# noway/nzcp-circom

Measured on NVIDIA B200. Metric: groth16_proofs_per_sec, higher is better.
Workload: dtype u256 (Fr/Fq Montgomery, 8x32-bit limbs, IMAD.WIDE carry chains)

## Files before the change

nzcp_circom_b200/csrc/msm.cu:

```cuda
#include <atomic>

#include "common.cuh"
#include "msm_pair.cuh"

#ifndef NZCP_G2_ACC_BLOCKS
#define NZCP_G2_ACC_BLOCKS 3
#endif

namespace nzcp {

#ifndef NZCP_TASK_LEN_MAX
#define NZCP_TASK_LEN_MAX 64
#endif
static constexpr int kTaskLenMax = NZCP_TASK_LEN_MAX;
static_assert((NZCP_TASK_LEN_MAX & (NZCP_TASK_LEN_MAX - 1)) == 0 && NZCP_TASK_LEN_MAX >= 8, "task length must be a power of two");
static constexpr int kTaskLenMin = 8;
#ifndef NZCP_TARGET_TASKS
#define NZCP_TARGET_TASKS (148 * 640)
#endif
static constexpr int kTargetTasks = NZCP_TARGET_TASKS;
#ifndef NZCP_HEAVY_TASKS
#define NZCP_HEAVY_TASKS 16
#endif
static constexpr int kHeavyTasks = NZCP_HEAVY_TASKS;
// ... 331 lines not shown
    for (int r = 0; r < C; r++) round_off[(size_t)r * pitch + n_buckets] = carry[r];
    flags[5] = carry[R];
  }
}

__global__ void __launch_bounds__(256)
msm_task_fill_kernel(const uint32_t* __restrict__ bcount, const uint32_t* __restrict__ offsets,
                     const uint32_t* __restrict__ task_off, uint2* __restrict__ tasks, uint32_t n_buckets,
                     const uint32_t* __restrict__ flags) {
  const uint32_t t = blockIdx.x * blockDim.x + threadIdx.x;
  if (t >= flags[2]) return;
  const uint32_t tl = flags[4];
  uint32_t lo = 0, hi = n_buckets;
  while (hi - lo > 1) {
    uint32_t mid = (lo + hi) >> 1;
    if (task_off[mid] <= t) lo = mid; else hi = mid;
  }
  (void)tl;
  const uint32_t k = task_off[lo + 1] - task_off[lo], j = t - task_off[lo];
  const uint32_t cnt = bcount[lo], base = cnt / k, rem = cnt % k;
  tasks[t] = make_uint2(offsets[lo] + j * base + (j < rem ? j : rem), base + (j < rem ? 1u : 0u));
}

template <class T>
__device__ __forceinline__ void prefetch_l1(const T* p) {
  asm volatile("prefetch.global.L1 [%0];" ::"l"(p));
  if (sizeof(T) > 64) asm volatile("prefetch.global.L1 [%0];" ::"l"(reinterpret_cast<const char*>(p) + 64));
}

template <class F> struct AccumOcc { static constexpr int kBlocks = 5; };
template <> struct AccumOcc<Fq2> { static constexpr int kBlocks = NZCP_G2_ACC_BLOCKS; };

template <class F>
__global__ void __launch_bounds__(128, AccumOcc<F>::kBlocks)
msm_accumulate_kernel(const Affine<F>* __restrict__ table, const uint32_t* __restrict__ entries,
                      const uint2* __restrict__ tasks, const uint32_t* __restrict__ flags, XYZZ<F>* __restrict__ partial, int pf) {
  uint32_t t = blockIdx.x * blockDim.x + threadIdx.x;
  if (t >= flags[2]) return;
  uint2 tk = tasks[t];
  XYZZ<F> acc = XYZZ<F>::inf();
  uint32_t e = entries[tk.x];
  if (pf & 1) prefetch_l1(table + (e & 0x7fffffffu));
  for (uint32_t k = 0; k < tk.y; k++) {
    uint32_t en = e;
    if (k + 1 < tk.y) {
      en = entries[tk.x + k + 1];
      if (pf & 1) prefetch_l1(table + (en & 0x7fffffffu));
    }
    Affine<F> q;
#if defined(__CUDA_ARCH__)
    if (sizeof(F) == sizeof(Fq) && (pf & 4)) q = gather_hinted<Affine<F>>(table + (e & 0x7fffffffu));
    else
#endif
      q = table[e & 0x7fffffffu];
    if (!q.is_inf()) xyzz_madd(acc, q, (e >> 31) != 0);
    e = en;
  }
  partial[t] = acc;
}

template <class F>
__global__ void __launch_bounds__(128, AccumOcc<F>::kBlocks)
msm_accumulate_pts_kernel(const Affine<F>* __restrict__ pts, const uint2* __restrict__ tasks,
                          const uint32_t* __restrict__ flags, XYZZ<F>* __restrict__ partial) {
  uint32_t t = blockIdx.x * blockDim.x + threadIdx.x;
  if (t >= flags[2]) return;
  uint2 tk = tasks[t];
  XYZZ<F> acc = XYZZ<F>::inf();
  for (uint32_t k = 0; k < tk.y; k++) {
    Affine<F> q = pts[tk.x + k];
    if (!q.is_inf()) xyzz_madd(acc, q, false);
  }
  partial[t] = acc;
}

static constexpr int kPairInvGroup = 32;
#ifndef NZCP_PAIR_FWD_BLOCKS
#define NZCP_PAIR_FWD_BLOCKS 1
#endif
template <class F, bool FROM_TABLE, int K>
__global__ void __launch_bounds__(128, (sizeof(F) == sizeof(Fq) ? NZCP_PAIR_FWD_BLOCKS : 1))
msm_pair_forward_kernel(const Affine<F>* __restrict__ src, const uint32_t* __restrict__ entries,
                        const uint32_t* __restrict__ off_in, const uint32_t* __restrict__ off_out, uint32_t n_buckets,
                        F* __restrict__ scratch, F* __restrict__ prod, int pf, Affine<F>* __restrict__ ops) {
  const uint32_t t = blockIdx.x * blockDim.x + threadIdx.x;
  PairSource<F, FROM_TABLE> ps{src, entries, pf};
  msm_pair_forward_body<F, FROM_TABLE, K>(t, gridDim.x * blockDim.x, ps, off_in, off_out, n_buckets, scratch, prod, ops);
}

template <class F, int K>
__global__ void __launch_bounds__(64)
msm_pair_invert_kernel(F* __restrict__ prod, const uint32_t* __restrict__ off_out, uint32_t n_buckets) {
  const uint32_t n_out = off_out[n_buckets];
  const uint32_t n_prod = pair_n_prod<K>(n_out);
  msm_pair_invert_body<F, kPairInvGroup>(blockIdx.x * blockDim.x + threadIdx.x, prod, n_prod);
}

template <class F, bool FROM_TABLE, int K>
__global__ void __launch_bounds__(128)
msm_pair_backward_kernel(const Affine<F>* __restrict__ src, const uint32_t* __restrict__ entries,
                         const uint32_t* __restrict__ off_in, const uint32_t* __restrict__ off_out, uint32_t n_buckets,
                         Affine<F>* __restrict__ dst, const F* __restrict__ scratch, const F* __restrict__ inv_prod, int pf,
                         const Affine<F>* __restrict__ ops) {
  const uint32_t t = blockIdx.x * blockDim.x + threadIdx.x;
  PairSource<F, FROM_TABLE> ps{src, entries, pf};
  msm_pair_backward_body<F, FROM_TABLE, K>(t, gridDim.x * blockDim.x, ps, off_in, off_out, n_buckets, dst, scratch, inv_prod,
                                           ops);
}

template <class T>
__device__ __forceinline__ T load_cg(const T* p) {
  static_assert(sizeof(T) % 16 == 0, "16-byte granules");
  T r;
  const uint4* s = reinterpret_cast<const uint4*>(p);
  uint4* d = reinterpret_cast<uint4*>(&r);
#pragma unroll
  for (int i = 0; i < (int)(sizeof(T) / 16); i++) d[i] = __ldcg(s + i);
  return r;
}

template <class T>
__device__ __forceinline__ T shfl_down_obj(const T& v, unsigned delta) {
  T r;
  const uint32_t* s = reinterpret_cast<const uint32_t*>(&v);
  uint32_t* d = reinterpret_cast<uint32_t*>(&r);
#pragma unroll
  for (int i = 0; i < (int)(sizeof(T) / 4); i++) d[i] = __shfl_down_sync(0xffffffffu, s[i], delta);
  return r;
}

template <class F>
__global__ void __launch_bounds__(128)
msm_combine_kernel(const uint32_t* __restrict__ task_off, const XYZZ<F>* __restrict__ partial,
                   XYZZ<F>* __restrict__ buckets, uint32_t n_buckets, uint32_t* __restrict__ heavy_list,
                   uint32_t* __restrict__ heavy_count) {
  const uint32_t b = blockIdx.x * blockDim.x + threadIdx.x;
  if (b >= n_buckets) return;
  const uint32_t t0 = task_off[b], nt = task_off[b + 1] - t0;
  if (nt > (uint32_t)kHeavyTasks) {
    heavy_list[atomicAdd(heavy_count, 1u)] = b;
    return;
  }
  XYZZ<F> acc = XYZZ<F>::inf();
  for (uint32_t j = 0; j < nt; j++) xyzz_add(acc, partial[t0 + j]);
  buckets[b] = acc;
}

__global__ void __launch_bounds__(1024)
msm_heavy_scan_kernel(const uint32_t* __restrict__ task_off, const uint32_t* __restrict__ heavy_list,
                      uint32_t* __restrict__ heavy_count, uint32_t* __restrict__ chunk_off) {
  __shared__ uint32_t sums[1024];
  const uint32_t n = heavy_count[0];
  const uint32_t per = (n + 1023) / 1024;
  const uint32_t b = threadIdx.x * per;
  const uint32_t e = b + per < n ? b + per : n;
  auto chunks = [&](uint32_t h) {
    uint32_t bk = heavy_list[h];
    return (task_off[bk + 1] - task_off[bk] + kHeavyChunk - 1) / kHeavyChunk;
  };
  uint32_t acc = 0;
  for (uint32_t h = b; h < e; h++) acc += chunks(h);
  sums[threadIdx.x] = acc;
  __syncthreads();
  for (int off = 1; off < 1024; off <<= 1) {
    uint32_t v = threadIdx.x >= (uint32_t)off ? sums[threadIdx.x - off] : 0;
    __syncthreads();
    sums[threadIdx.x] += v;
    __syncthreads();
  }
  uint32_t run = threadIdx.x ? sums[threadIdx.x - 1] : 0;
  for (uint32_t h = b; h < e; h++) {
    chunk_off[h] = run;
    run += chunks(h);
  }
  if (threadIdx.x == 1023) {
    chunk_off[n] = sums[1023];
    heavy_count[1] = sums[1023];
  }
}

template <class F>
__device__ __forceinline__ XYZZ<F> block_sum(XYZZ<F> acc, XYZZ<F>* sm) {
  sm[threadIdx.x] = acc;
  __syncthreads();
  for (uint32_t stride = blockDim.x / 2; stride >= 1; stride >>= 1) {
    if (threadIdx.x < stride) {
// ... 331 lines not shown
    const uint32_t n_ctr = nb * n_copies;
    DigitParams dp{n_copies, (uint32_t)n_points, s->table_free ? 0u : (uint32_t)s->n_points, s->c, s->n_windows,
                   (uint32_t)s->group_buckets, s->table_free ? (uint32_t)s->group_buckets : 0u, nb};
    const unsigned gp = div_up(n_points, 256);
    const size_t hist_bytes = (size_t)nb * sizeof(uint32_t);
    if (s->smem_hist) {
      NZCP_CUDA(cudaMemsetAsync(s->counts + n_ctr, 0, sizeof(uint32_t), st));
      msm_digits_smem_kernel<false><<<n_copies, sort_threads, hist_bytes, st>>>(scalars, dp, s->counts, nullptr, s->flags);
    } else {
      NZCP_CUDA(cudaMemsetAsync(s->counts, 0, (n_ctr + 1) * sizeof(uint32_t), st));
      msm_digits_kernel<false><<<gp, 256, 0, st>>>(scalars, dp, s->counts, nullptr, s->flags);
    }
    NZCP_LAUNCH_CHECK();
    const uint32_t n_scan = n_ctr + 1;
    const uint32_t n_blk = div_up(n_scan, kScanBlock);
    uint32_t* blk_sum = s->block_sums;
    uint32_t* blk_off = s->block_sums + (s->n_buckets * s->n_copies / kScanBlock + 2);
    msm_scan_sums_kernel<<<n_blk, 256, 0, st>>>(s->counts, blk_sum, n_scan);
    NZCP_LAUNCH_CHECK();
    msm_scan_kernel<false><<<1, 1024, 0, st>>>(blk_sum, blk_off, n_blk, s->flags + 3, s->flags);
    NZCP_LAUNCH_CHECK();
    msm_scan_apply_kernel<<<n_blk, 256, 0, st>>>(s->counts, blk_off, s->offsets, s->smem_hist ? nullptr : s->cursors, n_scan);
    NZCP_LAUNCH_CHECK();
    if (s->smem_hist)
      msm_digits_smem_kernel<true><<<n_copies, sort_threads, hist_bytes, st>>>(scalars, dp, s->offsets, s->entries, s->flags);
    else
      msm_digits_kernel<true><<<gp, 256, 0, st>>>(scalars, dp, s->cursors, s->entries, s->flags);
    NZCP_LAUNCH_CHECK();
    switch (s->rounds) {
      case 0: msm_round_plan_kernel<0><<<1, 1024, 0, st>>>(s->offsets, n_copies, nb, s->round_off, s->red_count, s->flags); break;
      case 1: msm_round_plan_kernel<1><<<1, 1024, 0, st>>>(s->offsets, n_copies, nb, s->round_off, s->red_count, s->flags); break;
      case 2: msm_round_plan_kernel<2><<<1, 1024, 0, st>>>(s->offsets, n_copies, nb, s->round_off, s->red_count, s->flags); break;
      default: msm_round_plan_kernel<3><<<1, 1024, 0, st>>>(s->offsets, n_copies, nb, s->round_off, s->red_count, s->flags); break;
    }
    NZCP_LAUNCH_CHECK();
    msm_scan_kernel<true><<<1, 1024, 0, st>>>(s->red_count, s->task_off, nb, s->flags + 2, s->flags);
    NZCP_LAUNCH_CHECK();
    msm_task_fill_kernel<<<div_up(s->max_tasks, 256), 256, 0, st>>>(s->red_count, s->round_off + (size_t)s->rounds * (nb + 1),
                                                                     s->task_off, s->tasks, nb, s->flags);
    NZCP_LAUNCH_CHECK();
  } else {
    NZCP_CUDA(cudaMemsetAsync(s->task_off, 0, (nb + 1) * sizeof(uint32_t), st));
  }
  NZCP_CUDA(cudaMemcpyAsync(s->flags_host, s->flags, 8 * sizeof(uint32_t), cudaMemcpyDeviceToHost, st));
}

uint32_t msm_sort_check(const MsmSort* s) {
  if (s->flags_host[1]) throw std::runtime_error("witness/scalar value is not a canonical field element (>= r)");
  return s->flags_host[3];
}

void msm_run_create(MsmRun* r, const MsmSort* sort, bool g2) {
  *r = MsmRun();
  r->g2 = g2;
  size_t psz = g2 ? sizeof(G2XYZZ) : sizeof(G1XYZZ);
  size_t tot = 0;
  if (g2) {
    NZCP_CUDA(cudaFuncSetAttribute(msm_combine_heavy_kernel<Fq2>, cudaFuncAttributeMaxDynamicSharedMemorySize,
                                   (int)(kHeavyThreads * sizeof(G2XYZZ))));
    NZCP_CUDA(cudaFuncSetAttribute(msm_combine_heavy2_kernel<Fq2>, cudaFuncAttributeMaxDynamicSharedMemorySize,
                                   (int)(kHeavyThreads * sizeof(G2XYZZ))));
    NZCP_CUDA(cudaFuncSetAttribute(msm_marginal_kernel<Fq2>, cudaFuncAttributeMaxDynamicSharedMemorySize,
                                   (int)(kMargThreads * sizeof(G2XYZZ))));
  }
  r->partial = dev_alloc<unsigned char>(sort->max_tasks * psz, &tot);
  r->buckets = dev_alloc<unsigned char>(sort->n_buckets * psz, &tot);
  r->n_groups = sort->n_groups;
  r->c = sort->c;
  r->marg = dev_alloc<unsigned char>((size_t)r->n_groups * kMaxDigits * 32 * psz, &tot);
  r->marg_done = dev_alloc<uint32_t>((size_t)r->n_groups * kMaxDigits, &tot);
  NZCP_CUDA(cudaMemset(r->marg_done, 0, (size_t)r->n_groups * kMaxDigits * sizeof(uint32_t)));
  r->result = dev_alloc<unsigned char>(psz, &tot);
  r->heavy_list = dev_alloc<uint32_t>(sort->n_buckets, &tot);
  r->heavy_count = dev_alloc<uint32_t>(2, &tot);
  r->chunk_off = dev_alloc<uint32_t>(sort->n_buckets + 1, &tot);
  r->chunk_partial = dev_alloc<unsigned char>((sort->max_tasks / kHeavyChunk + sort->n_buckets + 1) * psz, &tot);
  r->out = dev_alloc<unsigned char>((size_t)r->n_groups * (kMaxDigits + 1) * psz, &tot);
  NZCP_CUDA(cudaMallocHost(&r->out_host, (size_t)r->n_groups * (kMaxDigits + 1) * psz));
  memset(r->out_host, 0, (size_t)r->n_groups * (kMaxDigits + 1) * psz);
  r->n_digits = (sort->c - 1 + 4) / 5;
  NZCP_CUDA(cudaFuncSetAttribute(msm_sum_points_kernel<Fq2>, cudaFuncAttributeMaxDynamicSharedMemorySize,
                                 (int)(kHeavyThreads * sizeof(G2XYZZ))));
  if (sort->rounds > 0) {
    const size_t asz = g2 ? sizeof(G2Affine) : sizeof(G1Affine), fsz = asz / 2, pad = 128 * 64;
    r->round_pts[0] = dev_alloc<unsigned char>((sort->round_max[1] + pad) * asz, &tot);
    if (sort->rounds > 1) r->round_pts[1] = dev_alloc<unsigned char>((sort->round_max[2] + pad) * asz, &tot);
    r->round_prefix = dev_alloc<unsigned char>((sort->round_max[1] + pad) * fsz, &tot);
    if (g_tune_pair_stage.load())
      r->round_ops = dev_alloc<unsigned char>((sort->round_max[1] + pad) * 2 * asz, &tot);
    r->round_prod = dev_alloc<unsigned char>((sort->round_max[1] / 4 + pad) * fsz, &tot);
  }
  NZCP_CUDA(cudaEventCreate(&r->ev_acc0));
  NZCP_CUDA(cudaEventCreate(&r->ev_acc1));
  r->scratch_bytes = tot;
}

void msm_run_destroy(MsmRun* r) {
  cudaFree(r->partial);
  cudaFree(r->buckets);
  cudaFree(r->marg);
  cudaFree(r->marg_done);
  cudaFree(r->result);
  cudaFree(r->heavy_list);
  cudaFree(r->heavy_count);
  cudaFree(r->chunk_off);
  cudaFree(r->chunk_partial);
  cudaFree(r->out);
  cudaFree(r->round_pts[0]);
  cudaFree(r->round_pts[1]);
  cudaFree(r->round_prefix);
  cudaFree(r->round_ops);
  cudaFree(r->round_prod);
  if (r->out_host) cudaFreeHost(r->out_host);
  if (r->ev_acc0) cudaEventDestroy(r->ev_acc0);
  if (r->ev_acc1) cudaEventDestroy(r->ev_acc1);
  *r = MsmRun();
}

template <class F>
static void msm_run_launch_t(MsmRun* r, const MsmSort* s, const MsmTable* t, cudaStream_t st) {
  if (t->c != s->c || t->n_points != s->n_points || t->n_windows != (s->table_free ? 1 : s->n_windows))
    throw std::runtime_error("msm: table and sort plan do not match");
  const uint32_t nb = (uint32_t)s->n_buckets;
  const size_t psz = sizeof(XYZZ<F>);
  XYZZ<F>* partial = reinterpret_cast<XYZZ<F>*>(r->partial);
  XYZZ<F>* buckets = reinterpret_cast<XYZZ<F>*>(r->buckets);
  XYZZ<F>* out = reinterpret_cast<XYZZ<F>*>(r->out);
  NZCP_CUDA(cudaMemsetAsync(r->heavy_count, 0, 2 * sizeof(uint32_t), st));
  NZCP_CUDA(cudaEventRecord(r->ev_acc0, st));
  if (s->rounds == 0) {
    msm_accumulate_kernel<F><<<div_up(s->max_tasks, 128), 128, 0, st>>>(reinterpret_cast<const Affine<F>*>(t->pts),
                                                                       s->entries, s->tasks, s->flags, partial,
                                                                       (g_tune_acc_prefetch.load() ? 1 : 0) | (g_tune_gather_hint.load() ? 4 : 0));
    NZCP_LAUNCH_CHECK();
  } else {
    const Affine<F>* src = reinterpret_cast<const Affine<F>*>(t->pts);
    for (int rd = 1; rd <= s->rounds; rd++) {
      Affine<F>* dst = reinterpret_cast<Affine<F>*>(r->round_pts[(rd - 1) & 1]);
      const uint32_t* off_in = s->round_off + (size_t)(rd - 1) * (nb + 1);
      const uint32_t* off_out = s->round_off + (size_t)rd * (nb + 1);
      const int hint = g_tune_gather_hint.load() ? 4 : 0;
      const int pf_fwd = g_tune_pair_prefetch[0].load() | hint, pf_bwd = g_tune_pair_prefetch[1].load() | hint;
      int k = g_tune_pair_k[rd - 1].load();
      k = k >= 32 ? 32 : k >= 16 ? 16 : k >= 8 ? 8 : 4;
      const unsigned grid = div_up(div_up(s->round_max[rd], k) + kPairLanes, 128);
      const unsigned grid_inv = div_up(div_up((size_t)grid * 128, kPairInvGroup), 64);
      F* scratch = reinterpret_cast<F*>(r->round_prefix);
      F* prod = reinterpret_cast<F*>(r->round_prod);
      Affine<F>* ops = g_tune_pair_stage.load() ? reinterpret_cast<Affine<F>*>(r->round_ops) : nullptr;
#define NZCP_PAIR_LAUNCH(TABLE, KK)                                                                                       \
      do {                                                                                                                \
        msm_pair_forward_kernel<F, TABLE, KK><<<grid, 128, 0, st>>>(src, s->entries, off_in, off_out, nb, scratch, prod, \
                                                                    pf_fwd, TABLE ? ops : nullptr);                       \
        NZCP_LAUNCH_CHECK();                                                                                              \
        msm_pair_invert_kernel<F, KK><<<grid_inv, 64, 0, st>>>(prod, off_out, nb);                                        \
        NZCP_LAUNCH_CHECK();                                                                                              \
        msm_pair_backward_kernel<F, TABLE, KK><<<grid, 128, 0, st>>>(src, s->entries, off_in, off_out, nb, dst, scratch,  \
                                                                     prod, pf_bwd, TABLE ? ops : nullptr);                \
        NZCP_LAUNCH_CHECK();                                                                                              \
      } while (0)
      if (rd == 1) {
        if (k == 32) NZCP_PAIR_LAUNCH(true, 32); else if (k == 16) NZCP_PAIR_LAUNCH(true, 16);
        else if (k == 8) NZCP_PAIR_LAUNCH(true, 8); else NZCP_PAIR_LAUNCH(true, 4);
      } else {
        if (k == 32) NZCP_PAIR_LAUNCH(false, 32); else if (k == 16) NZCP_PAIR_LAUNCH(false, 16);
        else if (k == 8) NZCP_PAIR_LAUNCH(false, 8); else NZCP_PAIR_LAUNCH(false, 4);
      }
#undef NZCP_PAIR_LAUNCH
      src = dst;
    }
    msm_accumulate_pts_kernel<F><<<div_up(s->max_tasks, 128), 128, 0, st>>>(src, s->tasks, s->flags, partial);
    NZCP_LAUNCH_CHECK();
  }
  NZCP_CUDA(cudaEventRecord(r->ev_acc1, st));
  msm_combine_kernel<F><<<div_up(nb, 128), 128, 0, st>>>(s->task_off, partial, buckets, nb, r->heavy_list,
                                                                     r->heavy_count);
  NZCP_LAUNCH_CHECK();
  msm_heavy_scan_kernel<<<1, 1024, 0, st>>>(s->task_off, r->heavy_list, r->heavy_count, r->chunk_off);
  NZCP_LAUNCH_CHECK();
  XYZZ<F>* chunk_partial = reinterpret_cast<XYZZ<F>*>(r->chunk_partial);
  msm_combine_heavy_kernel<F><<<148 * 16, kHeavyThreads, kHeavyThreads * psz, st>>>(s->task_off, partial, r->heavy_list,
                                                                                    r->heavy_count, r->chunk_off, chunk_partial,
                                                                                    buckets);
  NZCP_LAUNCH_CHECK();
  msm_combine_heavy2_kernel<F><<<148, kHeavyThreads, kHeavyThreads * psz, st>>>(r->heavy_list, r->heavy_count, r->chunk_off,
                                                                                chunk_partial, buckets);
  NZCP_LAUNCH_CHECK();
  const uint32_t bits = (uint32_t)(s->c - 1);
  const uint32_t n_digits = (bits + 4) / 5;
  XYZZ<F>* marg = reinterpret_cast<XYZZ<F>*>(r->marg);
  msm_marginal_kernel<F><<<(unsigned)s->n_groups * n_digits * 32, kMargThreads, kMargThreads * psz, st>>>(buckets, marg, out,
                                                                                                      r->marg_done, bits, n_digits);
  NZCP_LAUNCH_CHECK();
  NZCP_CUDA(cudaMemcpyAsync(r->out_host, r->out, (size_t)s->n_groups * (n_digits + 1) * psz, cudaMemcpyDeviceToHost, st));
}

void msm_run_finish_device(MsmRun* r, cudaStream_t st) {
  if (r->g2)
    msm_finish_kernel<Fq2><<<1, 32, 0, st>>>(reinterpret_cast<const G2XYZZ*>(r->out), reinterpret_cast<G2XYZZ*>(r->result),
                                             (uint32_t)r->n_groups, (uint32_t)r->n_digits, r->c);
  else
    msm_finish_kernel<Fq><<<1, 32, 0, st>>>(reinterpret_cast<const G1XYZZ*>(r->out), reinterpret_cast<G1XYZZ*>(r->result),
                                            (uint32_t)r->n_groups, (uint32_t)r->n_digits, r->c);
  NZCP_LAUNCH_CHECK();
}

void msm_sum_points(const void* d_pts, uint32_t count, bool g2, void* d_result, cudaStream_t st) {
  if (g2) {
    NZCP_CUDA(cudaFuncSetAttribute(msm_sum_points_kernel<Fq2>, cudaFuncAttributeMaxDynamicSharedMemorySize,
                                   (int)(kHeavyThreads * sizeof(G2XYZZ))));
    msm_sum_points_kernel<Fq2><<<1, kHeavyThreads, kHeavyThreads * sizeof(G2XYZZ), st>>>(
        reinterpret_cast<const G2XYZZ*>(d_pts), count, reinterpret_cast<G2XYZZ*>(d_result));
  } else {
    msm_sum_points_kernel<Fq><<<1, kHeavyThreads, kHeavyThreads * sizeof(G1XYZZ), st>>>(
        reinterpret_cast<const G1XYZZ*>(d_pts), count, reinterpret_cast<G1XYZZ*>(d_result));
  }
  NZCP_LAUNCH_CHECK();
}

void msm_run_launch(MsmRun* r, const MsmSort* sort, const MsmTable* table, cudaStream_t st) {
  if (r->g2 != table->g2) throw std::runtime_error("msm: run and table group mismatch");
  if (r->g2)
    msm_run_launch_t<Fq2>(r, sort, table, st);
  else
    msm_run_launch_t<Fq>(r, sort, table, st);
}

template <class F>
static XYZZ<F> msm_run_finish_t(const MsmRun* r) {
  XYZZ<F> res = XYZZ<F>::inf();
  for (int g = r->n_groups - 1; g >= 0; g--) {
    const XYZZ<F>* w = reinterpret_cast<const XYZZ<F>*>(r->out_host) + (size_t)g * (r->n_digits + 1);
    XYZZ<F> acc = XYZZ<F>::inf();
    for (int k = r->n_digits - 1; k >= 0; k--) {
      if (!acc.is_inf())
        for (int d = 0; d < 5; d++) acc = xyzz_dbl(acc);
      xyzz_add(acc, w[k]);
    }
// ... 22 lines not shown
```

nzcp_circom_b200/csrc/msm_pair.cuh:

```cuda
#pragma once
#include "ec.cuh"


namespace nzcp {

enum PairKind { kPairNormal = 0, kPairDouble = 1, kPairFirst = 2, kPairSecond = 3, kPairInfinity = 4 };

#if defined(__CUDA_ARCH__)
template <class T>
__device__ __forceinline__ T gather_hinted(const T* p) {
  static_assert(sizeof(T) % 16 == 0, "16-byte granules");
  T r;
  uint4* d = reinterpret_cast<uint4*>(&r);
  const char* a = reinterpret_cast<const char*>(p);
#pragma unroll
  for (int i = 0; i < (int)(sizeof(T) / 16); i++)
    asm volatile("ld.global.nc.L2::64B.v4.u32 {%0, %1, %2, %3}, [%4];" : "=r"(d[i].x), "=r"(d[i].y), "=r"(d[i].z), "=r"(d[i].w) : "l"(a + 16 * i));
  return r;
}
#endif

template <class F, bool FROM_TABLE>
struct PairSource {
  const Affine<F>* pts;
  const uint32_t* entries;
  int pf = 0;
  HD uint32_t slot(uint32_t idx) const { return FROM_TABLE ? entries[idx] : idx; }
  HD F x_at(uint32_t slot) const {
#if defined(__CUDA_ARCH__)
    if (FROM_TABLE && (pf & 4)) return gather_hinted<F>(&pts[slot & 0x7fffffffu].x);
#endif
    return pts[FROM_TABLE ? (slot & 0x7fffffffu) : slot].x;
  }
  HD Affine<F> point_at(uint32_t slot) const {
    if (FROM_TABLE) {
      Affine<F> p;
#if defined(__CUDA_ARCH__)
      if (pf & 4) p = gather_hinted<Affine<F>>(&pts[slot & 0x7fffffffu]);
      else
#endif
        p = pts[slot & 0x7fffffffu];
      if (slot >> 31) p.y = f_neg(p.y);
      return p;
    }
    return pts[slot];
  }
  HD Affine<F> point(uint32_t idx) const { return point_at(slot(idx)); }
  HD void prefetch(uint32_t slot, bool whole_point) const {
#if defined(__CUDA_ARCH__)
    if ((pf & 3) == 0) return;
    const char* a = reinterpret_cast<const char*>(pts + (FROM_TABLE ? (slot & 0x7fffffffu) : slot));
    if ((pf & 3) == 1) {
      asm volatile("prefetch.global.L1 [%0];" ::"l"(a));
      if (sizeof(F) > 32 && whole_point) asm volatile("prefetch.global.L1 [%0];" ::"l"(a + 64));
    } else {
      asm volatile("prefetch.global.L2 [%0];" ::"l"(a));
      if (sizeof(F) > 32 && whole_point) asm volatile("prefetch.global.L2 [%0];" ::"l"(a + 64));
    }
#else
    (void)slot;
    (void)whole_point;
#endif
  }
};

struct PairWalk {
  const uint32_t* off_in;
  const uint32_t* off_out;
  uint32_t s, out0, out1, in0, len;
  HD void load() {
    out0 = off_out[s];
    out1 = off_out[s + 1];
    in0 = off_in[s];
    len = off_in[s + 1] - in0;
  }
  HD void forward_to(uint32_t o) {
    if (o < out1) return;
    do s++; while (o >= off_out[s + 1]);
    load();
  }
  HD void backward_to(uint32_t o) {
    if (o >= out0) return;
    do s--; while (o < off_out[s]);
    load();
  }
  HD uint32_t first(uint32_t o) const { return in0 + 2 * (o - out0); }
  HD bool paired(uint32_t o) const { return 2 * (o - out0) + 1 < len; }
};

template <class F>
HD int pair_classify(const Affine<F>& p1, const Affine<F>& p2, F& den) {
  if (p1.is_inf()) return kPairSecond;
  if (p2.is_inf()) return kPairFirst;
  den = f_sub(p2.x, p1.x);
  if (den.is_zero()) {
    if (p1.y == p2.y && !p1.y.is_zero()) {
      den = f_dbl(p1.y);
      return kPairDouble;
    }
    return kPairInfinity;
  }
  return kPairNormal;
}

static constexpr uint32_t kPairLanes = 32;
template <int K>
HD bool pair_thread_range(uint32_t t, const uint32_t* off_out, uint32_t n_buckets, uint32_t& o0, uint32_t& cnt) {
  const uint32_t n_out = off_out[n_buckets];
  const uint64_t first = (uint64_t)(t / kPairLanes) * (kPairLanes * K) + (t % kPairLanes);
  if (first >= n_out) return false;
  o0 = (uint32_t)first;
  const uint32_t left = (n_out - o0 + kPairLanes - 1) / kPairLanes;
  cnt = left < (uint32_t)K ? left : (uint32_t)K;
  return true;
}
template <int K>
HD uint32_t pair_n_prod(uint32_t n_out) {
  const uint32_t full = n_out / (kPairLanes * K), rem = n_out - full * (kPairLanes * K);
  return full * kPairLanes + (rem < kPairLanes ? rem : kPairLanes);
}
HD void pair_walk_seek(PairWalk& wk, uint32_t o, uint32_t n_buckets) {
  uint32_t lo = 0, hi = n_buckets;
  while (hi - lo > 1) {
    const uint32_t mid = (lo + hi) >> 1;
    if (wk.off_out[mid] <= o) lo = mid; else hi = mid;
  }
  wk.s = lo;
  wk.load();
}

template <class F, bool FROM_TABLE, int K>
HD void msm_pair_forward_body(uint32_t t, uint32_t stride, const PairSource<F, FROM_TABLE>& src, const uint32_t* off_in,
                              const uint32_t* off_out, uint32_t n_buckets, F* scratch, F* prod, Affine<F>* ops = nullptr) {
  uint32_t o0, cnt;
  if (!pair_thread_range<K>(t, off_out, n_buckets, o0, cnt)) return;
  PairWalk wk{off_in, off_out, 0, 0, 0, 0, 0};
  pair_walk_seek(wk, o0, n_buckets);
  F pre = F::one();
  bool have = false;
  bool pair_cur = wk.paired(o0);
  uint32_t a_cur = src.slot(wk.first(o0)), b_cur = pair_cur ? src.slot(wk.first(o0) + 1) : 0;
  for (uint32_t i = 0; i < cnt; i++) {
    bool pair_nxt = false;
    uint32_t a_nxt = 0, b_nxt = 0;
    if (i + 1 < cnt) {
      const uint32_t on = o0 + (i + 1) * kPairLanes;
      wk.forward_to(on);
      pair_nxt = wk.paired(on);
      if (pair_nxt || ops) a_nxt = src.slot(wk.first(on));
      if (pair_nxt) {
        b_nxt = src.slot(wk.first(on) + 1);
        src.prefetch(a_nxt, false);
        src.prefetch(b_nxt, false);
      }
    }
    if (ops) {
      const Affine<F> p1 = src.point_at(a_cur);
      const Affine<F> p2 = pair_cur ? src.point_at(b_cur) : Affine<F>::inf();
      ops[2 * ((size_t)i * stride + t)] = p1;
      ops[2 * ((size_t)i * stride + t) + 1] = p2;
      if (pair_cur) {
        F den;
        const int kind = pair_classify(p1, p2, den);
        if (kind == kPairNormal || kind == kPairDouble) {
          pre = have ? f_mul(pre, den) : den;
          have = true;
        }
      }
    } else if (pair_cur) {
      const F x1 = src.x_at(a_cur), x2 = src.x_at(b_cur);
      F den = f_sub(x2, x1);
      bool use = true;
      if (den.is_zero() || x1.is_zero() || x2.is_zero()) {
        const int kind = pair_classify(src.point_at(a_cur), src.point_at(b_cur), den);
        use = kind == kPairNormal || kind == kPairDouble;
      }
      if (use) {
        pre = have ? f_mul(pre, den) : den;
        have = true;
      }
    }
    scratch[(size_t)i * stride + t] = pre;
    pair_cur = pair_nxt;
    a_cur = a_nxt;
    b_cur = b_nxt;
  }
  prod[t] = pre;
}

template <class F, int KI>
HD void msm_pair_invert_body(uint32_t g, F* v, uint32_t n) {
  const uint32_t b = g * KI;
  if (b >= n) return;
  const uint32_t cnt = n - b < (uint32_t)KI ? n - b : (uint32_t)KI;
  F pre[KI];
  F run = v[b];
  pre[0] = run;
  for (uint32_t i = 1; i < cnt; i++) {
    run = f_mul(run, v[b + i]);
    pre[i] = run;
  }
  F inv = f_inv_fast(run);
  for (uint32_t i = cnt; i-- > 1;) {
    const F x = v[b + i];
    v[b + i] = f_mul(inv, pre[i - 1]);
    inv = f_mul(inv, x);
  }
  v[b] = inv;
}

template <class F>
HD Affine<F> pair_finish(const Affine<F>& p1, const Affine<F>& p2, F& inv, const F& before) {
  F den;
  const int kind = pair_classify(p1, p2, den);
  if (kind >= kPairFirst) return kind == kPairFirst ? p1 : kind == kPairSecond ? p2 : Affine<F>::inf();
  const F dinv = f_mul(inv, before);
  inv = f_mul(inv, den);
  F num;
  if (kind == kPairDouble) {
    const F xx = f_sqr(p1.x);
    num = f_add(f_dbl(xx), xx);
  } else {
    num = f_sub(p2.y, p1.y);
  }
  const F lam = f_mul(num, dinv);
  const F x3 = f_sub(f_sub(f_sqr(lam), p1.x), p2.x);
  const F y3 = f_sub(f_mul(lam, f_sub(p1.x, x3)), p1.y);
  return Affine<F>{x3, y3};
}

template <class F, bool FROM_TABLE, int K>
HD void msm_pair_backward_body(uint32_t t, uint32_t stride, const PairSource<F, FROM_TABLE>& src, const uint32_t* off_in,
                               const uint32_t* off_out, uint32_t n_buckets, Affine<F>* dst, const F* scratch,
                               const F* inv_prod, const Affine<F>* ops = nullptr) {
  uint32_t o0, cnt;
  if (!pair_thread_range<K>(t, off_out, n_buckets, o0, cnt)) return;
  if (ops) {
    F inv = inv_prod[t];
    for (uint32_t i = cnt; i-- > 0;) {
      const Affine<F> p1 = ops[2 * ((size_t)i * stride + t)], p2 = ops[2 * ((size_t)i * stride + t) + 1];
      const F before = i ? scratch[(size_t)(i - 1) * stride + t] : F::one();
      dst[o0 + i * kPairLanes] = pair_finish(p1, p2, inv, before);
    }
    return;
  }
  PairWalk wk{off_in, off_out, 0, 0, 0, 0, 0};
  pair_walk_seek(wk, o0 + (cnt - 1) * kPairLanes, n_buckets);
  F inv = inv_prod[t];
  bool pair_cur;
  uint32_t a_cur, b_cur;
  {
    const uint32_t o = o0 + (cnt - 1) * kPairLanes;
    pair_cur = wk.paired(o);
    a_cur = src.slot(wk.first(o));
    b_cur = pair_cur ? src.slot(wk.first(o) + 1) : 0;
  }
  for (uint32_t i = cnt; i-- > 0;) {
    const uint32_t o = o0 + i * kPairLanes;
    bool pair_nxt = false;
    uint32_t a_nxt = 0, b_nxt = 0;
    if (i > 0) {
      wk.backward_to(o - kPairLanes);
      pair_nxt = wk.paired(o - kPairLanes);
      a_nxt = src.slot(wk.first(o - kPairLanes));
      src.prefetch(a_nxt, true);
      if (pair_nxt) {
        b_nxt = src.slot(wk.first(o - kPairLanes) + 1);
        src.prefetch(b_nxt, true);
      }
    }
    if (!pair_cur) {
      dst[o] = src.point_at(a_cur);
    } else {
      const F before = i ? scratch[(size_t)(i - 1) * stride + t] : F::one();
      dst[o] = pair_finish(src.point_at(a_cur), src.point_at(b_cur), inv, before);
    }
    pair_cur = pair_nxt;
    a_cur = a_nxt;
    b_cur = b_nxt;
  }
}

}
```

nzcp_circom_b200/csrc/standalone.cu:

```cuda
#include <memory>

#include "api_util.cuh"
#include "msm_pair.cuh"

namespace nzcp {

extern std::atomic<int> g_tune_rounds;
extern std::atomic<int> g_tune_pair_stage;
extern std::atomic<int> g_tune_pair_k[kMsmMaxRounds];
extern std::atomic<int> g_tune_rounds_w, g_tune_rounds_h;

struct DevBuf {
  void* p = nullptr;
  explicit DevBuf(size_t bytes) { NZCP_CUDA(cudaMalloc(&p, bytes ? bytes : 16)); }
  ~DevBuf() { cudaFree(p); }
  template <class T> T* as() { return reinterpret_cast<T*>(p); }
};

struct Timer {
  cudaEvent_t a, b;
  cudaStream_t st;
  explicit Timer(cudaStream_t s) : st(s) {
    NZCP_CUDA(cudaEventCreate(&a));
    NZCP_CUDA(cudaEventCreate(&b));
// ... 265 lines not shown
                       : "r"(y));
        } else {
          asm volatile("mad.lo.cc.u32 %0, %8, %9, %0;\n\tmadc.hi.u32 %1, %8, %9, %1;\n\t"
                       "mad.lo.cc.u32 %2, %8, %9, %2;\n\tmadc.hi.u32 %3, %8, %9, %3;\n\t"
                       "mad.lo.cc.u32 %4, %8, %9, %4;\n\tmadc.hi.u32 %5, %8, %9, %5;\n\t"
                       "mad.lo.cc.u32 %6, %8, %9, %6;\n\tmadc.hi.u32 %7, %8, %9, %7;"
                       : "+r"(a0), "+r"(a1), "+r"(a2), "+r"(a3), "+r"(a4), "+r"(a5), "+r"(a6), "+r"(a7)
                       : "r"(x), "r"(y));
          asm volatile("add.cc.u32 %0, %0, %8;\n\taddc.cc.u32 %1, %1, %8;\n\taddc.cc.u32 %2, %2, %8;\n\taddc.u32 %3, %3, %8;\n\t"
                       "add.cc.u32 %4, %4, %8;\n\taddc.cc.u32 %5, %5, %8;\n\taddc.cc.u32 %6, %6, %8;\n\taddc.u32 %7, %7, %8;"
                       : "+r"(c0), "+r"(c1), "+r"(c2), "+r"(c3), "+r"(c4), "+r"(c5), "+r"(c6), "+r"(c7)
                       : "r"(y));
        }
      }
    }
    uint32_t sx = a0 ^ a1 ^ a2 ^ a3 ^ a4 ^ a5 ^ a6 ^ a7 ^ c0 ^ c1 ^ c2 ^ c3 ^ c4 ^ c5 ^ c6 ^ c7;
    if (sx == 0x12345678u) sink[0] = sx;
  } else {
    Fq a = Fq::one(), b = Fq::r2(), c = Fq::one();
    a.v[0] ^= t & 0xffff;
    c.v[1] ^= (seed + t) & 0xffff;
    for (int i = 0; i < iters; i++) {
      a = fp_mul(a, b);
      c = fp_mul(c, b);
    }
    if ((a.v[0] ^ c.v[0]) == 0x12345678u) sink[0] = a.v[1];
  }
}

template <int mode>
__global__ void __launch_bounds__(256) pipeprobe_kernel(int iters, uint32_t seed, uint32_t* sink) {
  uint32_t t = blockIdx.x * blockDim.x + threadIdx.x;
  uint32_t a0 = t, a1 = t + 1, a2 = t + 2, a3 = t + 3, a4 = t + 4, a5 = t + 5, a6 = t + 6, a7 = t + 7;
  uint32_t c0 = t, c1 = t ^ 1, c2 = t ^ 2, c3 = t ^ 3, c4 = t ^ 4, c5 = t ^ 5, c6 = t ^ 6, c7 = t ^ 7;
  double d0 = t, d1 = t + 0.5, d2 = t + 1.5, d3 = t + 2.5, d4 = t + 3.5, d5 = t + 4.5, d6 = t + 5.5, d7 = t + 6.5;
  const double fx = 1.0 + 1e-9 * (seed & 3), fy = 1e-3 * (1 + (t & 1));
  uint32_t x = seed | 1, y = seed + t;
  for (int i = 0; i < iters; i++) {
#pragma unroll
    for (int k = 0; k < 8; k++) {
      if (mode == 0) {
        asm volatile("fma.rn.f64 %0, %0, %8, %9;\n\tfma.rn.f64 %1, %1, %8, %9;\n\tfma.rn.f64 %2, %2, %8, %9;\n\t"
                     "fma.rn.f64 %3, %3, %8, %9;\n\tfma.rn.f64 %4, %4, %8, %9;\n\tfma.rn.f64 %5, %5, %8, %9;\n\t"
                     "fma.rn.f64 %6, %6, %8, %9;\n\tfma.rn.f64 %7, %7, %8, %9;"
                     : "+d"(d0), "+d"(d1), "+d"(d2), "+d"(d3), "+d"(d4), "+d"(d5), "+d"(d6), "+d"(d7)
                     : "d"(fx), "d"(fy));
      } else {
        asm volatile("mad.lo.cc.u32 %0, %8, %9, %0;\n\tmadc.hi.u32 %1, %8, %9, %1;\n\t"
                     "mad.lo.cc.u32 %2, %8, %9, %2;\n\tmadc.hi.u32 %3, %8, %9, %3;\n\t"
                     "mad.lo.cc.u32 %4, %8, %9, %4;\n\tmadc.hi.u32 %5, %8, %9, %5;\n\t"
                     "mad.lo.cc.u32 %6, %8, %9, %6;\n\tmadc.hi.u32 %7, %8, %9, %7;"
                     : "+r"(a0), "+r"(a1), "+r"(a2), "+r"(a3), "+r"(a4), "+r"(a5), "+r"(a6), "+r"(a7)
                     : "r"(x), "r"(y));
        if (mode == 1) {
          asm volatile("fma.rn.f64 %0, %0, %4, %5;\n\tfma.rn.f64 %1, %1, %4, %5;\n\tfma.rn.f64 %2, %2, %4, %5;\n\t"
                       "fma.rn.f64 %3, %3, %4, %5;"
                       : "+d"(d0), "+d"(d1), "+d"(d2), "+d"(d3) : "d"(fx), "d"(fy));
        } else if (mode == 2) {
          asm volatile("lop3.b32 %0, %0, %1, %8, 0xE8;\n\tlop3.b32 %1, %1, %2, %8, 0xE8;\n\t"
                       "lop3.b32 %2, %2, %3, %8, 0xE8;\n\tlop3.b32 %3, %3, %4, %8, 0xE8;\n\t"
                       "lop3.b32 %4, %4, %5, %8, 0xE8;\n\tlop3.b32 %5, %5, %6, %8, 0xE8;\n\t"
                       "lop3.b32 %6, %6, %7, %8, 0xE8;\n\tlop3.b32 %7, %7, %0, %8, 0xE8;"
                       : "+r"(c0), "+r"(c1), "+r"(c2), "+r"(c3), "+r"(c4), "+r"(c5), "+r"(c6), "+r"(c7) : "r"(y));
        } else {
          asm volatile("add.u32 %0, %0, %1;\n\tadd.u32 %1, %1, %2;\n\tadd.u32 %2, %2, %3;\n\tadd.u32 %3, %3, %4;\n\t"
                       "add.u32 %4, %4, %5;\n\tadd.u32 %5, %5, %6;\n\tadd.u32 %6, %6, %7;\n\tadd.u32 %7, %7, %0;"
                       : "+r"(c0), "+r"(c1), "+r"(c2), "+r"(c3), "+r"(c4), "+r"(c5), "+r"(c6), "+r"(c7));
        }
      }
    }
  }
  uint32_t sx = a0 ^ a1 ^ a2 ^ a3 ^ a4 ^ a5 ^ a6 ^ a7 ^ c0 ^ c1 ^ c2 ^ c3 ^ c4 ^ c5 ^ c6 ^ c7;
  double sd = d0 + d1 + d2 + d3 + d4 + d5 + d6 + d7;
  if (sx == 0x12345678u || sd == 0.123456) sink[0] = sx;
}


template <class F, int K>
static void sim_round(bool from_table, const std::vector<Affine<F>>& src, const std::vector<uint32_t>& entries,
                      const std::vector<uint32_t>& off_in, const std::vector<uint32_t>& off_out, uint32_t nb,
                      std::vector<Affine<F>>& dst, bool stage_ops) {
  const uint32_t n_out = off_out[nb];
  const uint32_t threads = pair_n_prod<K>(n_out) + 3;
  std::vector<F> scratch((size_t)threads * K), prod(threads + 40, F::one());
  std::vector<Affine<F>> ops(from_table && stage_ops ? (size_t)threads * K * 2 : 0);
  Affine<F>* opsp = ops.empty() ? nullptr : ops.data();
  dst.assign(n_out ? n_out : 1, Affine<F>::inf());
  const uint32_t n_prod = pair_n_prod<K>(n_out);
  for (int phase = 0; phase < 3; phase++) {
    if (phase == 1) {
      for (uint32_t g = 0; g * 32 < n_prod + 64; g++) msm_pair_invert_body<F, 32>(g, prod.data(), n_prod);
      continue;
    }
    for (uint32_t t = 0; t < threads; t++) {
      if (from_table) {
        PairSource<F, true> ps{src.data(), entries.data(), 0};
        if (phase == 0) msm_pair_forward_body<F, true, K>(t, threads, ps, off_in.data(), off_out.data(), nb, scratch.data(), prod.data(), opsp);
        else msm_pair_backward_body<F, true, K>(t, threads, ps, off_in.data(), off_out.data(), nb, dst.data(), scratch.data(), prod.data(), opsp);
      } else {
        PairSource<F, false> ps{src.data(), nullptr, 0};
        if (phase == 0) msm_pair_forward_body<F, false, K>(t, threads, ps, off_in.data(), off_out.data(), nb, scratch.data(), prod.data());
        else msm_pair_backward_body<F, false, K>(t, threads, ps, off_in.data(), off_out.data(), nb, dst.data(), scratch.data(), prod.data());
      }
    }
  }
}

template <class F>
static XYZZ<F> host_msm_sim(const uint8_t* bases, const uint8_t* scalars, size_t n, int c, int rounds, int k) {
  const int n_windows = msm_num_windows(c);
  const uint32_t nb = 1u << (c - 1);
  std::vector<Affine<F>> table((size_t)n_windows * n + 1);
  for (size_t i = 0; i < n; i++) {
    Affine<F> p;
    memcpy(&p, bases + i * sizeof(Affine<F>), sizeof(Affine<F>));
    table[i] = p;
    for (int w = 1; w < n_windows; w++) {
      if (!p.is_inf()) {
        XYZZ<F> acc = xyzz_dbl_affine(p);
        for (int j = 1; j < c; j++) acc = xyzz_dbl(acc);
        p = xyzz_to_affine(acc);
      }
      table[(size_t)w * n + i] = p;
    }
  }
  std::vector<std::vector<uint32_t>> lists(nb);
  for (size_t i = 0; i < n; i++) {
    uint32_t sc[8];
    memcpy(sc, scalars + 32 * i, 32);
    if (fp_geq_mod<FrParams>(sc)) throw ApiError(NZCP_E_RANGE, "witness/scalar value is not a canonical field element (>= r)");
    uint32_t carry = 0;
    for (int w = 0; w < n_windows; w++) {
      const int pos = w * c;
      uint32_t d = carry;
      if (pos < 256) {
        const int idx = pos >> 5, sh = pos & 31;
        uint64_t lo = sc[idx], hi = idx + 1 < 8 ? sc[idx + 1] : 0;
        d += (uint32_t)((lo | (hi << 32)) >> sh) & ((1u << c) - 1);
      }
      uint32_t neg = 0;
      if (d > nb) {
        d = (1u << c) - d;
        neg = 1;
        carry = 1;
      } else {
        carry = 0;
      }
      if (d) lists[d - 1].push_back(((uint32_t)w * (uint32_t)n + (uint32_t)i) | (neg << 31));
    }
  }
  std::vector<uint32_t> entries;
  std::vector<std::vector<uint32_t>> off(rounds + 1, std::vector<uint32_t>(nb + 1, 0));
  for (uint32_t b = 0; b < nb; b++) {
    uint32_t len = (uint32_t)lists[b].size();
    entries.insert(entries.end(), lists[b].begin(), lists[b].end());
    for (int r = 0; r <= rounds; r++) {
      off[r][b + 1] = off[r][b] + len;
      len = (len + 1) >> 1;
    }
  }
  entries.push_back(0);
  std::vector<Affine<F>> cur, nxt;
  const bool stage = g_tune_pair_stage.load() != 0;
  for (int r = 1; r <= rounds; r++) {
    const std::vector<Affine<F>>& src = r == 1 ? table : cur;
    switch (k) {
      case 4: sim_round<F, 4>(r == 1, src, entries, off[r - 1], off[r], nb, nxt, stage); break;
      case 16: sim_round<F, 16>(r == 1, src, entries, off[r - 1], off[r], nb, nxt, stage); break;
      case 32: sim_round<F, 32>(r == 1, src, entries, off[r - 1], off[r], nb, nxt, stage); break;
      case 8: sim_round<F, 8>(r == 1, src, entries, off[r - 1], off[r], nb, nxt, stage); break;
      default: throw ApiError(NZCP_E_ARG, "additions per thread must be 4, 8, 16 or 32");
    }
    cur.swap(nxt);
  }
// ... 306 lines not shown
```

Baseline: 131.4.

## Batch G2 pair inversions over Fq norms instead of Fq2 denominators

For G2 affine pair additions, the batched-inversion prefix products now run over the Fq norm of each Fq2 denominator (c0^2 + c1^2) rather than the Fq2 value itself. Each denominator's inverse is recovered as the conjugate scaled by the inverted norm. This halves scratch and prod storage per element and replaces Fq2 multiplications in the prefix chain and the inversion kernel with cheaper Fq ones. In exchange, each forward step computes two squarings and each backward step adds two multiplications plus a negation.

```diff
diff --git a/nzcp_circom_b200/csrc/msm.cu b/nzcp_circom_b200/csrc/msm.cu
--- a/nzcp_circom_b200/csrc/msm.cu
+++ b/nzcp_circom_b200/csrc/msm.cu
@@ -437,7 +437,8 @@
 __global__ void __launch_bounds__(128, (sizeof(F) == sizeof(Fq) ? NZCP_PAIR_FWD_BLOCKS : 1))
 msm_pair_forward_kernel(const Affine<F>* __restrict__ src, const uint32_t* __restrict__ entries,
                         const uint32_t* __restrict__ off_in, const uint32_t* __restrict__ off_out, uint32_t n_buckets,
-                        F* __restrict__ scratch, F* __restrict__ prod, int pf, Affine<F>* __restrict__ ops) {
+                        typename PairBatch<F>::Field* __restrict__ scratch, typename PairBatch<F>::Field* __restrict__ prod,
+                        int pf, Affine<F>* __restrict__ ops) {
   const uint32_t t = blockIdx.x * blockDim.x + threadIdx.x;
   PairSource<F, FROM_TABLE> ps{src, entries, pf};
   msm_pair_forward_body<F, FROM_TABLE, K>(t, gridDim.x * blockDim.x, ps, off_in, off_out, n_buckets, scratch, prod, ops);
@@ -455,8 +456,8 @@
 __global__ void __launch_bounds__(128)
 msm_pair_backward_kernel(const Affine<F>* __restrict__ src, const uint32_t* __restrict__ entries,
                          const uint32_t* __restrict__ off_in, const uint32_t* __restrict__ off_out, uint32_t n_buckets,
-                         Affine<F>* __restrict__ dst, const F* __restrict__ scratch, const F* __restrict__ inv_prod, int pf,
-                         const Affine<F>* __restrict__ ops) {
+                         Affine<F>* __restrict__ dst, const typename PairBatch<F>::Field* __restrict__ scratch,
+                         const typename PairBatch<F>::Field* __restrict__ inv_prod, int pf, const Affine<F>* __restrict__ ops) {
   const uint32_t t = blockIdx.x * blockDim.x + threadIdx.x;
   PairSource<F, FROM_TABLE> ps{src, entries, pf};
   msm_pair_backward_body<F, FROM_TABLE, K>(t, gridDim.x * blockDim.x, ps, off_in, off_out, n_buckets, dst, scratch, inv_prod,
@@ -954,7 +955,8 @@
   NZCP_CUDA(cudaFuncSetAttribute(msm_sum_points_kernel<Fq2>, cudaFuncAttributeMaxDynamicSharedMemorySize,
                                  (int)(kHeavyThreads * sizeof(G2XYZZ))));
   if (sort->rounds > 0) {
-    const size_t asz = g2 ? sizeof(G2Affine) : sizeof(G1Affine), fsz = asz / 2, pad = 128 * 64;
+    const size_t asz = g2 ? sizeof(G2Affine) : sizeof(G1Affine), pad = 128 * 64;
+    const size_t fsz = g2 ? sizeof(PairBatch<Fq2>::Field) : sizeof(PairBatch<Fq>::Field);
     r->round_pts[0] = dev_alloc<unsigned char>((sort->round_max[1] + pad) * asz, &tot);
     if (sort->rounds > 1) r->round_pts[1] = dev_alloc<unsigned char>((sort->round_max[2] + pad) * asz, &tot);
     r->round_prefix = dev_alloc<unsigned char>((sort->round_max[1] + pad) * fsz, &tot);
@@ -1017,15 +1019,16 @@
       k = k >= 32 ? 32 : k >= 16 ? 16 : k >= 8 ? 8 : 4;
       const unsigned grid = div_up(div_up(s->round_max[rd], k) + kPairLanes, 128);
       const unsigned grid_inv = div_up(div_up((size_t)grid * 128, kPairInvGroup), 64);
-      F* scratch = reinterpret_cast<F*>(r->round_prefix);
-      F* prod = reinterpret_cast<F*>(r->round_prod);
+      typedef typename PairBatch<F>::Field B;
+      B* scratch = reinterpret_cast<B*>(r->round_prefix);
+      B* prod = reinterpret_cast<B*>(r->round_prod);
       Affine<F>* ops = g_tune_pair_stage.load() ? reinterpret_cast<Affine<F>*>(r->round_ops) : nullptr;
 #define NZCP_PAIR_LAUNCH(TABLE, KK)                                                                                       \
       do {                                                                                                                \
         msm_pair_forward_kernel<F, TABLE, KK><<<grid, 128, 0, st>>>(src, s->entries, off_in, off_out, nb, scratch, prod, \
                                                                     pf_fwd, TABLE ? ops : nullptr);                       \
         NZCP_LAUNCH_CHECK();                                                                                              \
-        msm_pair_invert_kernel<F, KK><<<grid_inv, 64, 0, st>>>(prod, off_out, nb);                                        \
+        msm_pair_invert_kernel<B, KK><<<grid_inv, 64, 0, st>>>(prod, off_out, nb);                                        \
         NZCP_LAUNCH_CHECK();                                                                                              \
         msm_pair_backward_kernel<F, TABLE, KK><<<grid, 128, 0, st>>>(src, s->entries, off_in, off_out, nb, dst, scratch,  \
                                                                      prod, pf_bwd, TABLE ? ops : nullptr);                \
diff --git a/nzcp_circom_b200/csrc/msm_pair.cuh b/nzcp_circom_b200/csrc/msm_pair.cuh
--- a/nzcp_circom_b200/csrc/msm_pair.cuh
+++ b/nzcp_circom_b200/csrc/msm_pair.cuh
@@ -103,6 +103,21 @@
   return kPairNormal;
 }
 
+template <class F> struct PairBatch;
+template <> struct PairBatch<Fq> {
+  typedef Fq Field;
+  HD static Fq den_norm(const Fq& d) { return d; }
+  HD static Fq den_inverse(const Fq& d, const Fq& norm_inv) {
+    (void)d;
+    return norm_inv;
+  }
+};
+template <> struct PairBatch<Fq2> {
+  typedef Fq Field;
+  HD static Fq den_norm(const Fq2& d) { return fp_add(fp_sqr(d.c0), fp_sqr(d.c1)); }
+  HD static Fq2 den_inverse(const Fq2& d, const Fq& norm_inv) { return Fq2{fp_mul(d.c0, norm_inv), fp_neg(fp_mul(d.c1, norm_inv))}; }
+};
+
 static constexpr uint32_t kPairLanes = 32;
 template <int K>
 HD bool pair_thread_range(uint32_t t, const uint32_t* off_out, uint32_t n_buckets, uint32_t& o0, uint32_t& cnt) {
@@ -131,12 +146,14 @@
 
 template <class F, bool FROM_TABLE, int K>
 HD void msm_pair_forward_body(uint32_t t, uint32_t stride, const PairSource<F, FROM_TABLE>& src, const uint32_t* off_in,
-                              const uint32_t* off_out, uint32_t n_buckets, F* scratch, F* prod, Affine<F>* ops = nullptr) {
+                              const uint32_t* off_out, uint32_t n_buckets, typename PairBatch<F>::Field* scratch,
+                              typename PairBatch<F>::Field* prod, Affine<F>* ops = nullptr) {
+  typedef typename PairBatch<F>::Field B;
   uint32_t o0, cnt;
   if (!pair_thread_range<K>(t, off_out, n_buckets, o0, cnt)) return;
   PairWalk wk{off_in, off_out, 0, 0, 0, 0, 0};
   pair_walk_seek(wk, o0, n_buckets);
-  F pre = F::one();
+  B pre = B::one();
   bool have = false;
   bool pair_cur = wk.paired(o0);
   uint32_t a_cur = src.slot(wk.first(o0)), b_cur = pair_cur ? src.slot(wk.first(o0) + 1) : 0;
@@ -163,7 +180,8 @@
         F den;
         const int kind = pair_classify(p1, p2, den);
         if (kind == kPairNormal || kind == kPairDouble) {
-          pre = have ? f_mul(pre, den) : den;
+          const B n = PairBatch<F>::den_norm(den);
+          pre = have ? f_mul(pre, n) : n;
           have = true;
         }
       }
@@ -176,7 +194,8 @@
         use = kind == kPairNormal || kind == kPairDouble;
       }
       if (use) {
-        pre = have ? f_mul(pre, den) : den;
+        const B n = PairBatch<F>::den_norm(den);
+        pre = have ? f_mul(pre, n) : n;
         have = true;
       }
     }
@@ -210,12 +229,14 @@
 }
 
 template <class F>
-HD Affine<F> pair_finish(const Affine<F>& p1, const Affine<F>& p2, F& inv, const F& before) {
+HD Affine<F> pair_finish(const Affine<F>& p1, const Affine<F>& p2, typename PairBatch<F>::Field& inv,
+                         const typename PairBatch<F>::Field& before) {
   F den;
   const int kind = pair_classify(p1, p2, den);
   if (kind >= kPairFirst) return kind == kPairFirst ? p1 : kind == kPairSecond ? p2 : Affine<F>::inf();
-  const F dinv = f_mul(inv, before);
-  inv = f_mul(inv, den);
+  const typename PairBatch<F>::Field norm_inv = f_mul(inv, before);
+  inv = f_mul(inv, PairBatch<F>::den_norm(den));
+  const F dinv = PairBatch<F>::den_inverse(den, norm_inv);
   F num;
   if (kind == kPairDouble) {
     const F xx = f_sqr(p1.x);
@@ -231,22 +252,24 @@
 
 template <class F, bool FROM_TABLE, int K>
 HD void msm_pair_backward_body(uint32_t t, uint32_t stride, const PairSource<F, FROM_TABLE>& src, const uint32_t* off_in,
-                               const uint32_t* off_out, uint32_t n_buckets, Affine<F>* dst, const F* scratch,
-                               const F* inv_prod, const Affine<F>* ops = nullptr) {
+                               const uint32_t* off_out, uint32_t n_buckets, Affine<F>* dst,
+                               const typename PairBatch<F>::Field* scratch, const typename PairBatch<F>::Field* inv_prod,
+                               const Affine<F>* ops = nullptr) {
+  typedef typename PairBatch<F>::Field B;
   uint32_t o0, cnt;
   if (!pair_thread_range<K>(t, off_out, n_buckets, o0, cnt)) return;
   if (ops) {
-    F inv = inv_prod[t];
+    B inv = inv_prod[t];
     for (uint32_t i = cnt; i-- > 0;) {
       const Affine<F> p1 = ops[2 * ((size_t)i * stride + t)], p2 = ops[2 * ((size_t)i * stride + t) + 1];
-      const F before = i ? scratch[(size_t)(i - 1) * stride + t] : F::one();
+      const B before = i ? scratch[(size_t)(i - 1) * stride + t] : B::one();
       dst[o0 + i * kPairLanes] = pair_finish(p1, p2, inv, before);
     }
     return;
   }
   PairWalk wk{off_in, off_out, 0, 0, 0, 0, 0};
   pair_walk_seek(wk, o0 + (cnt - 1) * kPairLanes, n_buckets);
-  F inv = inv_prod[t];
+  B inv = inv_prod[t];
   bool pair_cur;
   uint32_t a_cur, b_cur;
   {
@@ -272,7 +295,7 @@
     if (!pair_cur) {
       dst[o] = src.point_at(a_cur);
     } else {
-      const F before = i ? scratch[(size_t)(i - 1) * stride + t] : F::one();
+      const B before = i ? scratch[(size_t)(i - 1) * stride + t] : B::one();
       dst[o] = pair_finish(src.point_at(a_cur), src.point_at(b_cur), inv, before);
     }
     pair_cur = pair_nxt;
diff --git a/nzcp_circom_b200/csrc/standalone.cu b/nzcp_circom_b200/csrc/standalone.cu
--- a/nzcp_circom_b200/csrc/standalone.cu
+++ b/nzcp_circom_b200/csrc/standalone.cu
@@ -371,14 +371,15 @@
                       std::vector<Affine<F>>& dst, bool stage_ops) {
   const uint32_t n_out = off_out[nb];
   const uint32_t threads = pair_n_prod<K>(n_out) + 3;
-  std::vector<F> scratch((size_t)threads * K), prod(threads + 40, F::one());
+  typedef typename PairBatch<F>::Field B;
+  std::vector<B> scratch((size_t)threads * K), prod(threads + 40, B::one());
   std::vector<Affine<F>> ops(from_table && stage_ops ? (size_t)threads * K * 2 : 0);
   Affine<F>* opsp = ops.empty() ? nullptr : ops.data();
   dst.assign(n_out ? n_out : 1, Affine<F>::inf());
   const uint32_t n_prod = pair_n_prod<K>(n_out);
   for (int phase = 0; phase < 3; phase++) {
     if (phase == 1) {
-      for (uint32_t g = 0; g * 32 < n_prod + 64; g++) msm_pair_invert_body<F, 32>(g, prod.data(), n_prod);
+      for (uint32_t g = 0; g * 32 < n_prod + 64; g++) msm_pair_invert_body<B, 32>(g, prod.data(), n_prod);
       continue;
     }
     for (uint32_t t = 0; t < threads; t++) {
```

New measurement: 132.1, median of 6. Within noise of the previous version (+0.5%).
